# hritikbharucha/Custom_Porechop_ABI

Hardware: AMD Instinct MI355X
Metric: reads/sec trimmed (100k ONT reads x 50 adapter pairs) (higher is better)
Workload: dtype int32

## Files before the change

### __graft_entry__.py

```python
import os
import subprocess
import sys

ROOT = os.path.dirname(os.path.abspath(__file__))
PKG = os.path.join(ROOT, 'custom_porechop_abi_amd')
HIPCC = os.environ.get('HIPCC', '/opt/rocm/bin/hipcc')


def _run(cmd, **kw):
    print('+', ' '.join(cmd), flush=True)
    subprocess.check_call(cmd, **kw)


def build_lib():
    from concurrent.futures import ThreadPoolExecutor
    csrc = os.path.join(PKG, 'csrc')
    out = os.path.join(PKG, 'libpcabi.so')
    bdir = os.path.join(ROOT, 'build')
    os.makedirs(bdir, exist_ok=True)
    hdr = os.path.join(ROOT, 'include', 'pcabi.h')
    dp, kern = os.path.join(csrc, 'pcabi_dp.h'), os.path.join(csrc, 'pcabi_kern.h')
    hip = [HIPCC, '--offload-arch=gfx950', '-O3', '-std=c++17', '-fPIC', '-Wall', '-c']
    hostdev = os.path.join(csrc, 'pcabi_hostdev.h')
    host = [dp, kern, hdr, os.path.join(csrc, 'pcabi_host.h'), os.path.join(csrc, 'pcabi_scratch.h'), hostdev]
    units = [(name, host, hip) for name in ('pcabi_engine.hip', 'pcabi_hostapi.hip', 'pcabi_middle.hip', 'pcabi_seed.hip')]
    units += [(name, [dp, kern, hdr], hip) for name in
             ('pcabi_k_packed_small.hip', 'pcabi_k_packed_large.hip', 'pcabi_k_fast.hip',
              'pcabi_k_chunk.hip', 'pcabi_k_aux.hip', 'pcabi_k_split.hip', 'pcabi_k_split_chunk.hip',
              'pcabi_k_group.hip', 'pcabi_cuts.hip', 'pcabi_decide.hip', 'pcabi_paths.hip')]
    defl, crc = os.path.join(csrc, 'pcabi_deflate.h'), os.path.join(csrc, 'pcabi_crc.h')
    infl = os.path.join(csrc, 'pcabi_inflate.h')
    bam = os.path.join(csrc, 'pcabi_bam.h')
    units += [('pcabi_kmer.hip', [os.path.join(csrc, 'pcabi_kmer.h'), hdr], hip),
              ('pcabi_deflate.hip', [defl, crc, hostdev, hdr], hip),
              ('pcabi_inflate.hip', [infl, defl, crc, hostdev, hdr], hip),
              ('pcabi_gzstream.hip', [os.path.join(csrc, 'pcabi_gzstream.h'), infl, defl, crc, hostdev, hdr], hip),
              ('pcabi_bam.hip', [bam, hostdev, hdr], hip),
              ('pcabi_mods.hip', [os.path.join(csrc, 'pcabi_mods.h'), bam, hostdev, hdr], hip),
              ('pcabi_moves.hip', [os.path.join(csrc, 'pcabi_moves.h'), hostdev, hdr], hip),
              ('pcabi_qual.hip', [os.path.join(csrc, 'pcabi_qual.h'), os.path.join(csrc, 'pcabi_pieces.h'), hostdev, hdr], hip),
              ('pcabi_auxtext.hip', [os.path.join(csrc, 'pcabi_auxtext.h'), hostdev, hdr], hip),
              ('pcabi_auxparse.hip', [os.path.join(csrc, 'pcabi_auxparse.h'), hostdev, hdr], hip)]
    reads, gxx = os.path.join(csrc, 'pcabi_reads.h'), ['g++', '-O3', '-std=c++17', '-fPIC', '-Wall', '-c']
    units += [('pcabi_io.cpp', [bam, reads, hostdev, hdr], gxx),
              ('pcabi_write.cpp', [defl, bam, os.path.join(csrc, 'pcabi_auxtext.h'), reads, hostdev, hdr], gxx)]

    def stale(target, deps):
        return not os.path.isfile(target) or any(os.path.getmtime(target) < os.path.getmtime(d) for d in deps)

    def compile_unit(u):
        name, deps, cmd = u
        src = os.path.join(csrc, name)
        obj = os.path.join(bdir, os.path.splitext(name)[0] + '.o')
        if stale(obj, [src] + deps):
            _run(cmd + ['-o', obj + '.tmp', src])
            os.replace(obj + '.tmp', obj)
        return obj

    jobs = int(os.environ.get('PCABI_BUILD_JOBS', min(8, os.cpu_count() or 1)))
    with ThreadPoolExecutor(max_workers=jobs) as ex:
        objs = list(ex.map(compile_unit, units))
    if stale(out, objs):
        _run([HIPCC, '--offload-arch=gfx950', '-shared', '-fPIC', '-o', out + '.tmp'] + objs + ['-lz'])
        os.replace(out + '.tmp', out)
    return out


def build_pystr():
    import sysconfig
    src = os.path.join(PKG, 'csrc', 'pystr.c')
    out = os.path.join(PKG, '_pystr' + sysconfig.get_config_var('EXT_SUFFIX'))
    if not os.path.isfile(out) or os.path.getmtime(out) < os.path.getmtime(src):
        _run(['gcc', '-O2', '-shared', '-fPIC', '-Wall', '-I', sysconfig.get_paths()['include'], '-o', out + '.tmp', src])
        os.replace(out + '.tmp', out)
    return out


# ... 48 lines not shown
```

### custom_porechop_abi_amd/csrc/pcabi_engine.hip

```cpp
#include <hip/hip_runtime.h>

#include <algorithm>
#include <atomic>
#include <cstdio>
#include <cstdlib>
#include <cstring>
#include <mutex>
#include <string>
#include <thread>
#include <vector>

#include "../../include/pcabi.h"
#include "pcabi_dp.h"
#include "pcabi_kern.h"
#include "pcabi_host.h"

namespace {
thread_local std::string g_err;
}

namespace pcabi_eng {
int fail(int code, const std::string &msg) {
    g_err = msg;
    return code;
}
}

using namespace pcabi_eng;

namespace {


int bucket_of(int L, const pcabi::Scoring &sc, bool allow_wide = true) {
    if (L > kMaxRPL) return kStripedBucket;
    if (L <= 64) {
        const int rpl = (L + 3) & ~3;
        if (pcabi::fast_ok(L, rpl, sc)) return rpl / 4 - 1;
    } else if (allow_wide && L <= pcabi::pk::MAX_L) {
        const int rpl = (L + 3) & ~3;
        if (pcabi::packed_ok(L, rpl, sc)) return 16 + (rpl - 68) / 4;
    } else if (allow_wide && L <= pcabi::pk::MAX_L_LONG) {
        const int b = L <= 96 ? 22 : (L <= 112 ? 23 : 24);
        if (pcabi::long_ok(L, kBuckets[b].rpl, sc)) return b;
    }
    if (L > 64 && sc.go != sc.ge) return kStripedBucket;
    for (int b = 0; b < kNumBuckets; ++b)
        if (kBuckets[b].kind == GENERIC && L <= kBuckets[b].rpl) return b;
    return -1;
}


struct EndFields {
    int rs, re, m, l1;
};
__device__ __forceinline__ EndFields end_fields(const int32_t *res, int64_t stride, int64_t i) {
    return EndFields{res[0 * stride + i], res[1 * stride + i], res[5 * stride + i], res[6 * stride + i]};
}

__global__ __launch_bounds__(256) void k_end_trim(const int32_t *sres, int64_t sstride, int32_t n_sa,
                                                  const int32_t *eres, int64_t estride, int32_t n_ea,
                                                  int64_t n_read, int end_size, int extra,
                                                  double thr, int min_trim,
                                                  int32_t *start_trim, int32_t *end_trim,
                                                  uint8_t *shit, uint8_t *ehit) {
    __shared__ int s_st[4][64], s_et[4][64];
    const int lane = threadIdx.x & 63, w = threadIdx.x >> 6;
    const int64_t r = (int64_t)blockIdx.x * 64 + lane;
// ... 615 lines not shown
}
int pcabi_event_destroy(void *ev) { HIP_TRY(hipEventDestroy((hipEvent_t)ev)); return 0; }
int pcabi_event_record(void *ev, void *stream) { HIP_TRY(hipEventRecord((hipEvent_t)ev, (hipStream_t)stream)); return 0; }
int pcabi_stream_wait_event(void *stream, void *ev) {
    HIP_TRY(hipStreamWaitEvent((hipStream_t)stream, (hipEvent_t)ev, 0));
    return 0;
}
int pcabi_event_elapsed_ms(float *ms, void *start, void *stop) {
    HIP_TRY(hipEventSynchronize((hipEvent_t)stop));
    HIP_TRY(hipEventElapsedTime(ms, (hipEvent_t)start, (hipEvent_t)stop));
    return 0;
}

}

namespace {
int adapters_create_impl(const uint8_t *adp_codes, const int32_t *adp_off, const int32_t *adp_len,
                         int32_t n_adp, const pcabi::Scoring *sc, pcabi_adapters **out, bool all_striped = false) {
    if (int rc = check_adapter_lens(adp_len, n_adp)) return rc;
    BucketHost bk[kNumBuckets];
    build_buckets(adp_codes, adp_off, adp_len, n_adp, sc ? *sc : pcabi::Scoring{1, -1, -1, -1}, bk, sc != nullptr,
                  sc != nullptr, all_striped);
    pcabi_adapters *a = new pcabi_adapters();
    a->n_adp = n_adp;
    a->hoff.resize((size_t)n_adp);
    a->hlen.assign(adp_len, adp_len + n_adp);
    for (int k = 0; k < n_adp; ++k) {
        a->hoff[k] = (int32_t)a->hcodes.size();
        for (int i = 0; i < adp_len[k]; ++i) {
            if (adp_codes[adp_off[k] + i] > 3) a->has_n = true;
            a->hcodes.push_back(adp_codes[adp_off[k] + i]);
        }
    }
    for (int b = 0; b < kNumBuckets; ++b) {
        const int nb = (int)bk[b].len.size();
        a->count[b] = nb;
        if (!nb) continue;
        a->lens[b] = bk[b].len;
        a->ids[b] = bk[b].id;
        a->rt[b] = bk[b].rt;
        for (int k = 0; k < nb; ++k) {
            if (bk[b].len[k] != kBuckets[b].rpl) a->padded[b] = true;
            a->max_off[b] = std::max(a->max_off[b], kBuckets[b].rpl - bk[b].len[k]);
        }
        const int64_t nw = (int64_t)bk[b].pad.size() / 4;
        if (a->pad[b].reserve(nw, nw) || a->len[b].reserve(nb, nb) || a->id[b].reserve(nb, nb)) {
            pcabi_adapters_destroy(a);
            return fail(PCABI_E_NOMEM, "hipMalloc failed for adapter table");
        }
        (void)hipMemcpy(a->pad[b], bk[b].pad.data(), bk[b].pad.size(), hipMemcpyHostToDevice);
        (void)hipMemcpy(a->len[b], bk[b].len.data(), sizeof(int32_t) * nb, hipMemcpyHostToDevice);
        (void)hipMemcpy(a->id[b], bk[b].id.data(), sizeof(int32_t) * nb, hipMemcpyHostToDevice);
    }
    *out = a;
    return 0;
}
}

bool layout_serves(const pcabi_adapters *adps, const pcabi::Scoring &sc, int64_t max_win) {
    int max_L = 0;
    bool regs = false;
    for (int b = 0; b < kNumBuckets; ++b) {
        if (!adps->count[b] || kBuckets[b].kind == STRIPED) continue;
        regs = true;
        for (int32_t L : adps->lens[b]) max_L = std::max<int>(max_L, L);
        if (kBuckets[b].kind == FAST && adps->padded[b] && !pcabi::fast_ok(kBuckets[b].rpl - 1, kBuckets[b].rpl, sc))
            return false;
        if (kBuckets[b].kind == FAST && adps->max_off[b] > 3 && !bucket_packed_ok(b, adps->lens[b], sc)) return false;
        if (kBuckets[b].kind == WIDE || kBuckets[b].kind == LONG)
            for (int32_t L : adps->lens[b])
                if (kBuckets[b].kind == WIDE ? !pcabi::packed_ok(L, kBuckets[b].rpl, sc)
                                             : !pcabi::long_ok(L, kBuckets[b].rpl, sc))
                    return false;
    }
    return !regs || !needs_striped(sc, max_L, max_win);
}

int adapters_for(const pcabi_adapters *adps, const pcabi::Scoring &sc, int64_t max_win, const pcabi_adapters **use) {
    if (layout_serves(adps, sc, max_win)) {
        *use = adps;
        return 0;
    }
    pcabi_adapters *a = const_cast<pcabi_adapters *>(adps);
    std::lock_guard<std::mutex> g(a->alt_mu);
    std::vector<int32_t> off((size_t)a->n_adp);
    for (int32_t k = 0; k < a->n_adp; ++k) off[k] = a->hoff[k];
    pcabi_adapters *t = nullptr;
    for (auto &e : a->alt_scored)
        if (e.first.ma == sc.ma && e.first.mi == sc.mi && e.first.go == sc.go && e.first.ge == sc.ge) t = e.second;
    if (!t) {
        if (int rc = adapters_create_impl(a->hcodes.data(), off.data(), a->hlen.data(), a->n_adp, &sc, &t)) return rc;
        a->alt_scored.emplace_back(sc, t);
    }
    if (layout_serves(t, sc, max_win)) {
        *use = t;
        return 0;
    }
    if (!a->alt_striped) {
        t = nullptr;
        if (int rc = adapters_create_impl(a->hcodes.data(), off.data(), a->hlen.data(), a->n_adp, &sc, &t, true))
            return rc;
        a->alt_striped = t;
    }
    *use = a->alt_striped;
    return 0;
}

static int record_event(void *ev, hipStream_t st) {
    HIP_TRY(hipEventRecord((hipEvent_t)ev, st));
    return 0;
}

static int bucket_params(const pcabi_adapters *t, int b, const pcabi::Scoring &sc, KParams &p) {
    p.adp_pad = t->pad[b];
    p.adp_len = t->len[b];
    p.adp_id = t->id[b];
    p.n_adp = t->count[b];
    p.rt = t->rt[b];
    const int pack = bucket_pack_mode(b, t->lens[b], sc);
    bucket_shift(b, t->lens[b], sc, pack, p);
    return pack;
}

extern "C" {

int pcabi_adapters_create(const uint8_t *adp_codes, const int32_t *adp_off, const int32_t *adp_len,
                          int32_t n_adp, pcabi_adapters **out) {
    return adapters_create_impl(adp_codes, adp_off, adp_len, n_adp, nullptr, out);
}

int pcabi_adapters_create_scored(const uint8_t *adp_codes, const int32_t *adp_off, const int32_t *adp_len,
                                 int32_t n_adp, int match, int mismatch, int gap_open, int gap_extend,
                                 pcabi_adapters **out) {
    const pcabi::Scoring sc{match, mismatch, gap_open, gap_extend};
    return adapters_create_impl(adp_codes, adp_off, adp_len, n_adp, &sc, out);
}

void pcabi_adapters_destroy(pcabi_adapters *a) {
    if (!a) return;
    for (auto &e : a->alt_scored) pcabi_adapters_destroy(e.second);
    pcabi_adapters_destroy(a->alt_striped);
    delete a;
}

int64_t pcabi_tile_layout(const int32_t *win_len, int64_t n_win, int64_t *tile_off) {
    if (n_win < 0 || !win_len || !tile_off) return fail(PCABI_E_ARG, "bad arguments");
    return tile_layout(win_len, n_win, tile_off, nullptr);
}

int pcabi_tile_windows_dev(const uint8_t *codes, const int64_t *win_off, const int32_t *win_len,
                           int64_t n_win, const int64_t *tile_off, int64_t max_chunks, uint32_t *tiles,
                           void *stream) {
    if (n_win < 0) return fail(PCABI_E_ARG, "bad arguments");
    launch_tiles(codes, win_off, win_len, n_win, tile_off, max_chunks, tiles, (hipStream_t)stream);
    HIP_TRY(hipGetLastError());
    return 0;
}

int pcabi_align_cross_dev(const uint32_t *tiles, const int64_t *tile_off, const int32_t *win_len,
                          int64_t n_win, int32_t max_win_len, const pcabi_adapters *adps, int match,
                          int mismatch, int gap_open, int gap_extend, int32_t *out, int64_t out_stride,
                          void *stream) {
    return pcabi_align_cross_dev_marked(tiles, tile_off, win_len, n_win, max_win_len, adps, match, mismatch,
                                        gap_open, gap_extend, out, out_stride, stream, nullptr, nullptr);
}

int pcabi_align_cross_dev_marked(const uint32_t *tiles, const int64_t *tile_off, const int32_t *win_len,
                                 int64_t n_win, int32_t max_win_len, const pcabi_adapters *adps, int match,
                                 int mismatch, int gap_open, int gap_extend, int32_t *out, int64_t out_stride,
                                 void *stream, void *ev_begin, void *ev_end) {
    if (!adps || n_win < 0 || (n_win > 0 && (!tiles || !tile_off))) return fail(PCABI_E_ARG, "bad arguments");
    if (n_win == 0) return 0;
    if (int rc = adapters_for(adps, pcabi::Scoring{match, mismatch, gap_open, gap_extend}, max_win_len, &adps))
        return rc;
    KParams p{};
    p.tiles = tiles;
    p.tile_off = tile_off;
    p.win_len = win_len;
    p.n_win = n_win;
    p.out = out;
    p.out_stride = out_stride;
    p.sc = pcabi::Scoring{match, mismatch, gap_open, gap_extend};
    p.max_cols = max_win_len;
    const bool affine = gap_open != gap_extend;
    std::vector<int> order;
    for (int b = 0; b < kNumBuckets; ++b)
        if (adps->count[b]) order.push_back(b);
    std::stable_sort(order.begin(), order.end(), [&](int x, int y) {
        return (int64_t)adps->count[x] * kBuckets[x].rpl > (int64_t)adps->count[y] * kBuckets[y].rpl;
    });
    ForkJoin fj;
    if (int rc = fj.begin((hipStream_t)stream, order.size())) return rc;
    for (size_t k = 0; k < order.size(); ++k) {
        const int b = order[k];
        const int pack = bucket_params(adps, b, p.sc, p);
        const hipStream_t st = fj.at(k);
        int rc = k == 0 && ev_begin ? record_event(ev_begin, st) : 0;
        if (!rc) rc = dispatch(b, p, affine, st, pack);
        if (!rc && k == 0 && ev_end) rc = record_event(ev_end, st);
        if (rc) {
            (void)fj.end();
            return rc;
        }
    }
    if (int rc = fj.end()) return rc;
    HIP_TRY(hipGetLastError());
    return 0;
}

int pcabi_align_cross_multi_dev(const pcabi_cross_region *regions, int32_t n_regions, int match, int mismatch,
                                int gap_open, int gap_extend, void *stream, void *ev_begin, void *ev_end) {
    if (n_regions < 0 || (n_regions > 0 && !regions)) return fail(PCABI_E_ARG, "bad arguments");
    const pcabi::Scoring sc{match, mismatch, gap_open, gap_extend};
    const bool affine = gap_open != gap_extend;
    struct Unit {
        int cls, b, pack;
        KParams p;
        int64_t blocks, cost;
    };
    std::vector<Unit> units;
    for (int32_t r = 0; r < n_regions; ++r) {
        const pcabi_cross_region &g = regions[r];
        if (!g.adps || g.n_win < 0 || (g.n_win > 0 && (!g.tiles || !g.tile_off || !g.win_len || !g.out)))
            return fail(PCABI_E_ARG, "bad region " + std::to_string(r));
        if (g.n_win == 0) continue;
        const pcabi_adapters *adps = nullptr;
        if (int rc = adapters_for(g.adps, sc, g.max_win_len, &adps)) return rc;
        for (int b = 0; b < kNumBuckets; ++b) {
            if (!adps->count[b]) continue;
            Unit u{};
            u.b = b;
            KParams &p = u.p;
            p.tiles = g.tiles;
            p.tile_off = g.tile_off;
            p.win_len = g.win_len;
            p.n_win = g.n_win;
            p.out = g.out;
            p.out_stride = g.out_stride;
            p.sc = sc;
            p.max_cols = g.max_win_len;
            u.pack = bucket_params(adps, b, sc, p);
            u.cls = kBuckets[b].kind == FAST ? group_class(kBuckets[b].rpl, u.pack, affine) : -1;
            u.blocks = (g.n_win + 8 * 256 - 1) / (8 * 256) * 8 * (int64_t)p.n_adp;
            u.cost = (g.n_win + 255) / 256 * (int64_t)p.n_adp * kBuckets[b].rpl;
            units.push_back(u);
        }
    }
    if (units.empty()) return 0;
    struct Launch {
        int cls;
        size_t unit;
        GroupParams gp;
        int64_t blocks, cost;
    };
    std::vector<Launch> launches;
    for (int c = 0; c < kGroupClasses; ++c) {
        std::vector<size_t> mine;
        for (size_t k = 0; k < units.size(); ++k)
            if (units[k].cls == c) mine.push_back(k);
        if (mine.size() == 1) units[mine[0]].cls = -1;
        if (mine.size() <= 1) continue;
        std::stable_sort(mine.begin(), mine.end(),
                         [&](size_t x, size_t y) { return kBuckets[units[x].b].rpl > kBuckets[units[y].b].rpl; });
        for (size_t k0 = 0; k0 < mine.size(); k0 += kMaxGroupSegs) {
            Launch l{};
            l.cls = c;
            l.gp.sc = sc;
            for (size_t k = k0; k < std::min(mine.size(), k0 + kMaxGroupSegs); ++k) {
                const Unit &u = units[mine[k]];
                GroupSeg &s = l.gp.seg[l.gp.n_seg++];
                s.tiles = u.p.tiles;
                s.tile_off = u.p.tile_off;
                s.win_len = u.p.win_len;
                s.n_win = u.p.n_win;
                s.adp_pad = u.p.adp_pad;
                s.adp_len = u.p.adp_len;
                s.adp_id = u.p.adp_id;
                s.n_adp = u.p.n_adp;
                s.out = u.p.out;
                s.out_stride = u.p.out_stride;
                s.rpl = kBuckets[u.b].rpl;
                s.shift_p = u.p.shift_p;
                s.shift_b = u.p.shift_b;
                s.block0 = l.blocks;
                l.blocks += u.blocks;
                l.cost += u.cost;
            }
            launches.push_back(l);
        }
    }
    for (size_t k = 0; k < units.size(); ++k)
        if (units[k].cls < 0) {
            Launch l{};
            l.cls = -1;
            l.unit = k;
            l.cost = units[k].cost;
            launches.push_back(l);
        }
    std::stable_sort(launches.begin(), launches.end(), [](const Launch &x, const Launch &y) { return x.cost > y.cost; });
    ForkJoin fj;
    if (int rc = fj.begin((hipStream_t)stream, launches.size())) return rc;
    for (size_t k = 0; k < launches.size(); ++k) {
        const Launch &l = launches[k];
        const hipStream_t st = fj.at(k);
        int rc = k == 0 && ev_begin ? record_event(ev_begin, st) : 0;
        if (!rc && l.cls >= 0) dispatch_group(l.cls, l.gp, l.blocks, st);
        else if (!rc) rc = dispatch(units[l.unit].b, units[l.unit].p, affine, st, units[l.unit].pack);
        if (!rc && k == 0 && ev_end) rc = record_event(ev_end, st);
        if (rc) {
            (void)fj.end();
            return rc;
        }
    }
    if (int rc = fj.end()) return rc;
    HIP_TRY(hipGetLastError());
    return 0;
}

int pcabi_set_side_streams(int on) {
    const int prev = side_streams_on() ? 1 : 0;
    if (on >= 0) g_side_on.store(on ? 1 : 0);
    return prev;
}

int pcabi_stream_side_streams(void *stream, int on) {
    const hipStream_t st = (hipStream_t)stream;
    std::lock_guard<std::mutex> g(g_stream_side_mu);
    for (size_t k = 0; k < g_stream_side.size(); ++k)
        if (g_stream_side[k].first == st) {
            const int prev = g_stream_side[k].second;
// ... 58 lines not shown
```

### custom_porechop_abi_amd/csrc/pcabi_host.h

```cpp
#pragma once

#include <hip/hip_runtime.h>

#include <atomic>
#include <mutex>
#include <utility>
#include <vector>

#include "../../include/pcabi.h"
#include "pcabi_dp.h"
#include "pcabi_kern.h"
#include "pcabi_scratch.h"

using pcabi_internal::Scratch;

void pcabi_poison_async(void *p, size_t bytes, hipStream_t st);

extern std::atomic<uint64_t> g_table_serial;
struct pcabi_adapters {
    int32_t n_adp = 0;
    uint64_t serial = g_table_serial.fetch_add(1) + 1;
    int rt[pcabi_eng::kNumBuckets] = {};
    bool padded[pcabi_eng::kNumBuckets] = {};
    int max_off[pcabi_eng::kNumBuckets] = {};
    std::vector<int32_t> lens[pcabi_eng::kNumBuckets];
    std::vector<int32_t> ids[pcabi_eng::kNumBuckets];
    bool has_n = false;
    std::vector<uint8_t> hcodes;
    std::vector<int32_t> hoff, hlen;
    int32_t count[pcabi_eng::kNumBuckets] = {};
    pcabi_internal::DevBuf<uint32_t> pad[pcabi_eng::kNumBuckets];
    pcabi_internal::DevBuf<int32_t> len[pcabi_eng::kNumBuckets], id[pcabi_eng::kNumBuckets];
    std::mutex alt_mu;
    std::vector<std::pair<pcabi::Scoring, pcabi_adapters *>> alt_scored;
    pcabi_adapters *alt_striped = nullptr;
};
bool layout_serves(const pcabi_adapters *adps, const pcabi::Scoring &sc, int64_t max_win);
int adapters_for(const pcabi_adapters *adps, const pcabi::Scoring &sc, int64_t max_win, const pcabi_adapters **use);

namespace pcabi_eng {

struct SideStreams;
struct ForkJoin {
    hipStream_t main = nullptr;
    SideStreams *ss = nullptr;
    std::unique_lock<std::mutex> lock;
    int first = 0;
    unsigned used = 0;
    int n_side = 0;
    int begin(hipStream_t m, size_t n_launch);
    hipStream_t at(size_t k);
    int end();
};

int64_t tile_layout(const int32_t *win_len, int64_t n_win, int64_t *tile_off, int64_t *max_nq);
void launch_tiles(const uint8_t *codes, const int64_t *win_off, const int32_t *win_len, int64_t n_win,
                  const int64_t *tile_off, int64_t max_nq, uint32_t *tiles, hipStream_t st);
int first_hit_from(const int32_t *res, int64_t stride, int64_t n_win, int32_t n_adp, double threshold,
                   const int32_t *start_adp, int32_t *hits, int64_t hit_stride, hipStream_t st);
void scan_set_table(pcabi_scan *s, const pcabi_adapters *adps);
bool chunkable(int b, bool packed);
int dispatch(int b, const KParams &p, bool affine, hipStream_t st, int packed);
bool bucket_packed_ok(int b, const std::vector<int32_t> &lens, const pcabi::Scoring &sc);
int bucket_pack_mode(int b, const std::vector<int32_t> &lens, const pcabi::Scoring &sc);
void bucket_shift(int b, const std::vector<int32_t> &lens, const pcabi::Scoring &sc, int pack_mode, KParams &p);

struct BucketHost {
    std::vector<uint8_t> pad;
    std::vector<int32_t> len, id;
    int rt = 0;
};
void build_buckets(const uint8_t *adp_codes, const int32_t *adp_off, const int32_t *adp_len, int32_t n_adp,
                   const pcabi::Scoring &sc, BucketHost (&bk)[kNumBuckets], bool merge = true, bool allow_wide = true,
                   bool all_striped = false);
int check_adapter_lens(const int32_t *adp_len, int32_t n_adp);
bool needs_striped(const pcabi::Scoring &sc, int max_L, int64_t max_win);

}

namespace pcabi_seed {
struct State;
State *create();
void destroy(State *s);
int bounds(State *s, const void *adps_key, const uint8_t *hcodes, const int32_t *hoff, const int32_t *hlen,
           int32_t n_adp, const std::vector<int> &fb_rows, const uint8_t *codes, const int64_t *v_off,
// ... 22 lines not shown
```

### custom_porechop_abi_amd/csrc/pcabi_k_group.hip

```cpp
#include "pcabi_kern.h"

namespace pcabi_eng {

template <int CLS>
__global__ __launch_bounds__(256) void k_align_group(GroupParams gp) {
    constexpr int MAXR = group_max_rpl(CLS);
    __shared__ __attribute__((aligned(16))) int32_t tab[4 * kTabW * MAXR];
    int32_t *wave_tab = tab + (threadIdx.x >> 6) * kTabW * MAXR;
    const int64_t b = blockIdx.x;
    int s = 0;
    while (s + 1 < gp.n_seg && b >= gp.seg[s + 1].block0) ++s;
    const GroupSeg &g = gp.seg[s];
    KParams p{};
    p.tiles = g.tiles;
    p.tile_off = g.tile_off;
    p.win_len = g.win_len;
    p.n_win = g.n_win;
    p.adp_pad = g.adp_pad;
    p.adp_len = g.adp_len;
    p.adp_id = g.adp_id;
    p.n_adp = g.n_adp;
    p.out = g.out;
    p.out_stride = g.out_stride;
    p.sc = gp.sc;
    p.shift_p = g.shift_p;
    p.shift_b = g.shift_b;
    const int64_t lb = b - g.block0;
    if constexpr (CLS == 0) {
        if (g.shift_p > 0) {
            switch (g.rpl) {
#define T(R) case R: cross_block<R, true, SHIFT>(p, lb, wave_tab); break;
            T(4) T(8) T(12) T(16) T(20) T(24) T(28) T(32)
#undef T
            }
        } else {
            switch (g.rpl) {
#define T(R) case R: cross_block<R, true, TAGGED>(p, lb, wave_tab); break;
            T(4) T(8) T(12) T(16) T(20) T(24) T(28) T(32)
#undef T
            }
        }
    } else {
        if (g.shift_p > 0) {
            switch (g.rpl) {
#define P(R) case R: cross_block<R, true, PSHIFT>(p, lb, wave_tab); break;
            P(36) P(40) P(44) P(48) P(52) P(56) P(60) P(64)
#undef P
            }
        } else {
            switch (g.rpl) {
#define P(R) case R: cross_block<R, true, PACKED>(p, lb, wave_tab); break;
            P(36) P(40) P(44) P(48) P(52) P(56) P(60) P(64)
#undef P
            }
        }
    }
}

void dispatch_group(int cls, const GroupParams &p, int64_t blocks, hipStream_t st) {
    if (blocks <= 0) return;
    if (cls == 0) hipLaunchKernelGGL((k_align_group<0>), dim3((unsigned)blocks), dim3(256), 0, st, p);
    else hipLaunchKernelGGL((k_align_group<1>), dim3((unsigned)blocks), dim3(256), 0, st, p);
}

}
```

### custom_porechop_abi_amd/csrc/pcabi_kern.h

```cpp
#pragma once
#include <hip/hip_runtime.h>

#include <algorithm>
#include <cstdint>
#include <cstdlib>
#include <string>
#include <type_traits>

#include "../../include/pcabi.h"
#include "pcabi_dp.h"

#ifndef PCABI_WAVES
#define PCABI_WAVES 1
#endif

void pcabi_poison(void *p, size_t bytes);
void pcabi_poison_async(void *p, size_t bytes, hipStream_t st);

namespace pcabi_eng {

int fail(int code, const std::string &msg);

#define HIP_TRY(expr)                                                                   \
    do {                                                                                \
        hipError_t e_ = (expr);                                                         \
        if (e_ != hipSuccess)                                                           \
            return fail(PCABI_E_DEVICE, std::string(#expr) + ": " + hipGetErrorString(e_)); \
    } while (0)

enum Kind { FAST = 0, GENERIC = 1, PACKED = 2, WIDE = 3, LONG = 4, STRIPED = 5,
            TAGGED = 6,
            SHIFT = 7,
            PSHIFT = 8 };
struct BucketDef {
    int rpl;
    Kind kind;
};
constexpr BucketDef kBuckets[] = {
    {4, FAST},  {8, FAST},  {12, FAST}, {16, FAST}, {20, FAST}, {24, FAST}, {28, FAST}, {32, FAST},
    {36, FAST}, {40, FAST}, {44, FAST}, {48, FAST}, {52, FAST}, {56, FAST}, {60, FAST}, {64, FAST},
    {68, WIDE}, {72, WIDE}, {76, WIDE}, {80, WIDE}, {84, WIDE}, {88, WIDE},
    {96, LONG}, {112, LONG}, {128, LONG},
    {16, GENERIC}, {32, GENERIC}, {64, GENERIC}, {96, GENERIC}, {128, GENERIC},
    {256, STRIPED}};
constexpr int kNumBuckets = sizeof(kBuckets) / sizeof(kBuckets[0]);
constexpr int kStripedBucket = kNumBuckets - 1;
constexpr int kMaxRPL = 128;
constexpr int kStripeRows = 32;
constexpr int kStripeTab = 64;

struct KParams {
    const uint8_t *codes;
    const int64_t *win_off;
    const int32_t *win_len;
    int64_t n_win;
    const uint32_t *tiles;
    const int64_t *tile_off;
    const uint32_t *adp_pad;
    const int32_t *adp_len;
    const int32_t *adp_id;
    int32_t n_adp;
    const int32_t *task_win;
    const int32_t *task_out;
    const int32_t *wave_adp;
    int64_t n_waves;
    int32_t *out;
    int64_t out_stride;
    pcabi::Scoring sc;
    int32_t *compat;
    int32_t chunk_split;
    const int4 *task_chunk;
    int32_t rt;
    int32_t max_cols;
    int32_t *scratch;
    int64_t n_items;
    const int32_t *dev_waves;
    int32_t shift_p, shift_b;
};

struct WindowReader {
    const uint32_t *q;
    int64_t stride;
    int a8;
    uint32_t lo, hi, nx;
    __device__ __forceinline__ WindowReader() : q(nullptr), stride(0), a8(0), lo(0), hi(0), nx(0) {}
    __device__ __forceinline__ WindowReader(const uint32_t *base, int64_t stride_, int a8_)
        : q(base), stride(stride_), a8(a8_) {
        lo = q[0]; hi = q[stride]; nx = q[2 * stride];
    }
    __device__ __forceinline__ int operator()(int j) {
        const int k = j - 1;
        if (k > 0 && (k & 3) == 0) { lo = hi; hi = nx; nx = q[(int64_t)(k / 4 + 2) * stride]; }
        return (int)(((((uint64_t)hi << 32) | lo) >> (8 * (k & 3) + a8)) & 0xFFu);
    }
};

template <int RPL>
struct AdapterRegs {
    uint32_t w[RPL / 4];
    __device__ __forceinline__ void load(const uint32_t *src) {
#pragma unroll
        for (int k = 0; k < RPL / 4; ++k) w[k] = __builtin_amdgcn_readfirstlane(src[k]);
    }
    __device__ __forceinline__ int operator()(int s) const {
        return (int)((w[(s - 1) >> 2] >> (8 * ((s - 1) & 3))) & 0xFFu);
    }
};

__device__ __forceinline__ void store_result(int32_t *out, int64_t stride, int64_t idx,
                                             const pcabi::Result &r) {
    out[0 * stride + idx] = r.rs;
    out[1 * stride + idx] = r.re;
    out[2 * stride + idx] = r.as;
    out[3 * stride + idx] = r.ae;
    out[4 * stride + idx] = r.score;
    out[5 * stride + idx] = r.m;
    out[6 * stride + idx] = r.l1;
    out[7 * stride + idx] = r.l2;
}

__device__ __forceinline__ pcabi::Result empty_result() {
    pcabi::Result r;
    r.rs = -1; r.re = 0; r.as = -1; r.ae = 0;
    r.score = (int)0x80000000; r.m = 0; r.l1 = 0; r.l2 = 0;
    return r;
}

constexpr int kTabW = pcabi::pk::TAB_W;

struct LdsRow {
    const int32_t *p;
    __device__ __forceinline__ int32_t operator()(int s) const { return p[s - 1]; }
    __device__ __forceinline__ void quad(int q, int32_t *dst) const {
        const int4 v = *reinterpret_cast<const int4 *>(p + 4 * q);
        dst[0] = v.x; dst[1] = v.y; dst[2] = v.z; dst[3] = v.w;
    }
};

template <int RPL, typename Y = pcabi::pk::Lay<RPL>>
__device__ __forceinline__ void fill_wave_tab(const KParams &p, int a_local, int L, int32_t *wave_tab) {
    const int off = RPL - L;
    const int lane = threadIdx.x & 63;
    for (int e = lane; e < kTabW * RPL; e += 64) {
        const int c = e / RPL, srow = e % RPL + 1;
        const uint32_t *ap = p.adp_pad + (int64_t)a_local * (RPL / 4);
        auto code = [&](int sl) { return (int)((ap[(sl - 1) / 4] >> (8 * ((sl - 1) & 3))) & 0xFFu); };
        wave_tab[e] = pcabi::pk::sub_key<RPL, decltype(code), Y>(srow, c, code, off, p.sc);
    }
    __syncthreads();
}

template <int RPL>
__device__ __forceinline__ void fill_wave_tab_shift(const KParams &p, int a_local, int L, int32_t *wave_tab) {
    const int off = RPL - L;
    const int lane = threadIdx.x & 63;
    for (int e = lane; e < kTabW * RPL; e += 64) {
        const int c = e / RPL, srow = e % RPL + 1;
        const uint32_t *ap = p.adp_pad + (int64_t)a_local * (RPL / 4);
        auto code = [&](int sl) { return (int)((ap[(sl - 1) / 4] >> (8 * ((sl - 1) & 3))) & 0xFFu); };
        wave_tab[e] = pcabi::pk::sub_key_shift<RPL>(srow, c, code, off, p.sc);
    }
    __syncthreads();
}

template <int RPL>
__device__ __forceinline__ void fill_wave_tab_pshift(const KParams &p, int a_local, int L, int32_t *wave_tab) {
    const int off = RPL - L;
    const int lane = threadIdx.x & 63;
    for (int e = lane; e < kTabW * RPL; e += 64) {
        const int c = e / RPL, srow = e % RPL + 1;
        const uint32_t *ap = p.adp_pad + (int64_t)a_local * (RPL / 4);
// ... 43 lines not shown
            auto tr = [&](int q) { return base[(int64_t)q * 256]; };
            auto tabfn = [&](int rc) { return LdsRow{wave_tab + rc * RPL}; };
            r = pcabi::align_lane_shift4<RPL>(tr, n0, tabfn, L, p.sc, P, p.shift_b);
            uniform = true;
        }
    }
    if (uniform) {
    } else if (n <= 0) {
        r = empty_result();
    } else {
        WindowReader rd = tile_off >= 0
            ? WindowReader(p.tiles + tile_off + (threadIdx.x & 255), 256, 0)
            : [&] {
                  const uint8_t *b = p.codes + p.win_off[w];
                  const int a0 = (int)((uintptr_t)b & 3);
                  return WindowReader(reinterpret_cast<const uint32_t *>(b - a0), 1, 8 * a0);
              }();
        if constexpr (KIND == PACKED) {
            auto tabfn = [&](int rc) { return LdsRow{wave_tab + rc * RPL}; };
            r = pcabi::align_lane_packed<(RPL <= pcabi::pk::MAX_RPL ? RPL : 4), AFFINE>(rd, n, tabfn, L, p.sc);
        } else if constexpr (KIND == TAGGED) {
            static_assert(RPL <= 32 && AFFINE, "run-tagged layout: affine buckets of <= 32 rows");
            auto tabfn = [&](int rc) { return LdsRow{wave_tab + rc * RPL}; };
            r = pcabi::align_lane_packed<RPL, true, false, pcabi::pk::LayT<RPL>>(rd, n, tabfn, L, p.sc);
        } else if constexpr (KIND == SHIFT) {
            static_assert(RPL <= 32 && AFFINE, "gap-extend frame: affine buckets of <= 32 rows");
            auto tabfn = [&](int rc) { return LdsRow{wave_tab + rc * RPL}; };
            r = pcabi::align_lane_shift<RPL>(rd, n, tabfn, L, p.sc, p.shift_p, p.shift_b);
        } else if constexpr (KIND == PSHIFT) {
            static_assert(RPL >= 36 && RPL <= 64 && AFFINE, "packed gap-extend frame: affine buckets of 36..64 rows");
            auto tabfn = [&](int rc) { return LdsRow{wave_tab + rc * RPL}; };
            r = pcabi::align_lane_pshift<RPL>(rd, n, tabfn, L, p.sc, p.shift_p, p.shift_b);
        } else if constexpr (KIND == LONG) {
            WindowReader rd1 = rd;
            auto tab0 = [&](int rc) { return LdsRow{wave_tab + rc * RPL}; };
            auto tab1 = [&](int rc) { return LdsRow{wave_tab + kTabW * RPL + rc * RPL}; };
            r = pcabi::align_lane_packed_long<RPL, AFFINE>(rd, rd1, n, tab0, tab1, L, p.sc);
        } else if constexpr (KIND == FAST) {
            r = pcabi::align_lane_fast<RPL, AFFINE>(rd, n, adp, L, p.sc);
        } else {
            r = pcabi::align_lane_generic<RPL, AFFINE>(rd, n, adp, L, p.sc);
        }
    }
    if (p.compat) {
        int en_match = 0;
        if (r.rs >= 0 && r.diag_en && r.l1 > 0) {
            const uint8_t *ab = reinterpret_cast<const uint8_t *>(p.adp_pad + (int64_t)a_local * (RPL / 4));
            en_match = p.codes[p.win_off[w] + r.re] == ab[RPL - L + r.ae];
        }
        p.compat[out_idx] = pcabi::compat_flag(r, n, en_match);
        return;
    }
    store_result(p.out, p.out_stride, out_idx, r);
}

template <int KIND, int RPL>
constexpr int wave_tab_ints() {
    return (KIND == PACKED || KIND == TAGGED || KIND == SHIFT || KIND == PSHIFT) ? kTabW * RPL : (KIND == LONG ? 2 * kTabW * RPL : 1);
}

template <int RPL, bool AFFINE, int KIND>
__device__ __forceinline__ void cross_block(const KParams &p, int64_t b, int32_t *wave_tab) {
    const int64_t k = b >> 3;
    const int a_local = (int)(k % p.n_adp);
    const int64_t tile = (k / p.n_adp) * 8 + (b & 7);
    const int64_t w = tile * 256 + threadIdx.x;
    const int a_glob = p.adp_id[a_local];
    const int64_t toff = w < p.n_win ? p.tile_off[tile] : 0;
    run_lane<RPL, AFFINE, KIND>(p, a_local, w < p.n_win ? w : -1, (int64_t)a_glob * p.n_win + w, wave_tab, toff);
}

template <int RPL, bool AFFINE, int KIND>
__global__ __launch_bounds__(256, PCABI_WAVES) void k_align(KParams p) {
    __shared__ __attribute__((aligned(16))) int32_t tab[4 * wave_tab_ints<KIND, RPL>()];
    int32_t *wave_tab = tab + (threadIdx.x >> 6) * wave_tab_ints<KIND, RPL>();
    if (p.task_win == nullptr) {
        cross_block<RPL, AFFINE, KIND>(p, blockIdx.x, wave_tab);
    } else {
        int64_t wave = (int64_t)blockIdx.x * 4 + (threadIdx.x >> 6);
        const bool live = wave < p.n_waves;
        if (!live) wave = p.n_waves - 1;
        const int64_t slot = wave * 64 + (threadIdx.x & 63);
        const int a_local = __builtin_amdgcn_readfirstlane(p.wave_adp[wave]);
        const int32_t tw = live ? p.task_win[slot] : -1;
        run_lane<RPL, AFFINE, KIND>(p, a_local, tw, tw >= 0 ? p.task_out[slot] : 0, wave_tab, -1);
    }
}

struct FParams {
    const uint32_t *tiles;
    const int64_t *tile_off;
    const int32_t *win_len;
    int64_t n_win;
    const uint32_t *adp_pad;
    const int32_t *adp_len;
    const int32_t *adp_id;
    int32_t n_adp;
    int16_t *s16;
    pcabi::Scoring sc;
};

struct LdsRow16 {
    const int32_t *p;
    __device__ __forceinline__ void quad(int q, pcabi::sf::v2 *dst) const {
        const int4 v = *reinterpret_cast<const int4 *>(p + 4 * q);
        dst[0] = __builtin_bit_cast(pcabi::sf::v2, v.x);
// ... 139 lines not shown

template <int R, bool AFFINE>
__global__ __launch_bounds__(256) void k_align_striped(KParams p) {
    const int64_t slot = (int64_t)blockIdx.x * 4 + (threadIdx.x >> 6);
    const int lane = threadIdx.x & 63;
    const int64_t n_slots = (int64_t)gridDim.x * 4;
    StripeBnd<AFFINE> bnd{p.scratch + slot * (int64_t)p.max_cols * (StripeBnd<AFFINE>::NF * 64) + lane};
    for (int64_t item = slot; item < p.n_items; item += n_slots) {
        const bool cross = p.task_win == nullptr;
        int a_local;
        int64_t w, out_idx, q = 0;
        int4 ck = make_int4(0, 0, 1, -1);
        if (cross) {
            a_local = (int)(item % p.n_adp);
            q = item / p.n_adp;
            w = q * 64 + lane;
            if (w >= p.n_win) continue;
            out_idx = (int64_t)p.adp_id[a_local] * p.n_win + w;
        } else {
            a_local = p.wave_adp[item];
            const int64_t sl = item * 64 + lane;
            w = p.task_win[sl];
            if (w < 0) continue;
            out_idx = p.task_out[sl];
            if (p.task_chunk) ck = p.task_chunk[sl];
        }
        a_local = __builtin_amdgcn_readfirstlane(a_local);
        const int L = __builtin_amdgcn_readfirstlane(p.adp_len[a_local]);
        const int n = p.task_chunk ? ck.y : p.win_len[w];
        pcabi::Result r;
        if (n <= 0) {
            r = empty_result();
        } else {
            WindowReader rd = cross
                ? WindowReader(p.tiles + p.tile_off[q >> 2] + (q & 3) * 64 + lane, 256, 0)
                : [&] {
                      const uint8_t *b = p.codes + p.win_off[w] + ck.x;
                      const int a0 = (int)((uintptr_t)b & 3);
                      return WindowReader(reinterpret_cast<const uint32_t *>(b - a0), 1, 8 * a0);
                  }();
            StripeAdp<R> adp{p.adp_pad + (int64_t)a_local * (p.rt / 4)};
            r = pcabi::align_lane_striped<R, AFFINE>(rd, n, adp, L, p.rt, p.sc, bnd, ck.z, ck.w);
        }
        if (p.compat) {
            int en_match = 0;
            if (r.rs >= 0 && r.diag_en && r.l1 > 0) {
                const uint8_t *ab = reinterpret_cast<const uint8_t *>(p.adp_pad + (int64_t)a_local * (p.rt / 4));
                en_match = p.codes[p.win_off[w] + r.re] == ab[p.rt - L + r.ae];
            }
            p.compat[out_idx] = pcabi::compat_flag(r, n, en_match);
            continue;
        }
        store_result(p.out, p.out_stride, out_idx, r);
    }
}

__device__ __forceinline__ int32_t lane_from_below(int32_t v) {
    return __builtin_amdgcn_update_dpp(0, v, 0x111, 0xF, 0xF, false);
}

template <int RPL, int K, bool AFFINE, int KIND>
__global__ __launch_bounds__(256, PCABI_WAVES) void k_align_split(KParams p) {
    constexpr int R = RPL / K;
    static_assert(RPL % K == 0 && 16 % K == 0 && R >= 2, "split geometry");
    using Y = typename std::conditional<KIND == TAGGED, pcabi::pk::LayT<RPL>, pcabi::pk::Lay<RPL>>::type;
    __shared__ __attribute__((aligned(16))) int32_t tab[4 * kTabW * RPL];
    int32_t *wave_tab = tab + (threadIdx.x >> 6) * (kTabW * RPL);
    const int64_t b = blockIdx.x;
    const int64_t k = b >> 3;
    const int a_local = (int)(k % p.n_adp);
    const int64_t q = k / p.n_adp;
    const int64_t tile = (q / K) * 8 + (b & 7);
    const int l = (int)(threadIdx.x % K);
    const int64_t w = tile * 256 + (q % K) * (256 / K) + threadIdx.x / K;
    const int L = __builtin_amdgcn_readfirstlane(p.adp_len[a_local]);
    fill_wave_tab<RPL, Y>(p, a_local, L, wave_tab);
    const bool live = w < p.n_win;
    const int n = live ? p.win_len[w] : 0;
    int nmax = n;
#pragma unroll
    for (int o = 1; o < 64; o <<= 1) nmax = max(nmax, __shfl_xor(nmax, o));
    WindowReader rd;
    if (n > 0) rd = WindowReader(p.tiles + p.tile_off[tile] + (w & 255), 256, 0);
    pcabi::LaneSplit<R, AFFINE, Y> st;
    st.init(l, K, L, RPL, p.sc);
    int32_t sg = st.gbot, sv = st.vbot;
    const int steps = nmax - 1 + K - 1;
#pragma unroll 1
    for (int t = 1; t <= steps; ++t) {
        int32_t rg = lane_from_below(sg), rv = lane_from_below(sv);
        if (l == 0) {
            rg = st.row0_g(t);
            rv = st.neg2;
        }
        const int j = t - l;
        if (j >= 1 && j < n) {
            const int c = rd(j);
            st.inner(LdsRow{wave_tab + c * RPL + st.r0}, j, rg, rv);
            sg = st.gbot;
            sv = st.vbot;
        }
    }
    st.out = pcabi::SplitIn{};
#pragma unroll
    for (int ph = 0; ph < K; ++ph) {
        pcabi::SplitIn in;
        in.gup = lane_from_below(st.out.gup);
        in.vup = lane_from_below(st.out.vup);
        in.slt = lane_from_below(st.out.slt);
        in.vt = lane_from_below(st.out.vt);
        in.vp = lane_from_below(st.out.vp);
        in.score = lane_from_below(st.out.score);
        in.bi = lane_from_below(st.out.bi);
        in.lt = lane_from_below(st.out.lt);
        in.trail = lane_from_below(st.out.trail);
        in.prec = lane_from_below(st.out.prec);
        in.attr = (uint32_t)lane_from_below((int32_t)st.out.attr);
        if (l == ph && n > 0) {
            if (l == 0) in = st.empty_in(n);
            const int c = rd(n);
            st.last_col(LdsRow{wave_tab + c * RPL + st.r0}, n, in);
        }
    }
    if (l == K - 1 && live)
        store_result(p.out, p.out_stride, (int64_t)p.adp_id[a_local] * p.n_win + w, n > 0 ? st.result(n) : empty_result());
}

template <int RPL, int K, bool AFFINE, int KIND>
__device__ __forceinline__ void split_chunk_wave(const KParams &p, int64_t pw, int sub, bool live, int32_t *wave_tab) {
    constexpr int R = RPL / K;
    using Y = typename std::conditional<KIND == TAGGED, pcabi::pk::LayT<RPL>, pcabi::pk::Lay<RPL>>::type;
    const int lane = threadIdx.x & 63, l = lane % K;
    const int64_t slot = pw * 64 + sub * (64 / K) + lane / K;
    const int a_local = __builtin_amdgcn_readfirstlane(p.wave_adp[pw]);
    const int L = __builtin_amdgcn_readfirstlane(p.adp_len[a_local]);
    fill_wave_tab<RPL, Y>(p, a_local, L, wave_tab);
    const int32_t tw = live ? p.task_win[slot] : -1;
    int4 ck = make_int4(0, 0, 1, 0);
    if (tw >= 0) ck = p.task_chunk[slot];
    const int n = tw >= 0 ? ck.y : 0;
    const bool at_end = ck.w < 0;
    const int hi = at_end ? n + 1 : ck.w;
    const int n_in = at_end ? n - 1 : n;
    int nmax = n_in;
#pragma unroll
    for (int o = 1; o < 64; o <<= 1) nmax = max(nmax, __shfl_xor(nmax, o));
    WindowReader rd;
    if (n > 0) {
        const uint8_t *b = p.codes + p.win_off[tw] + ck.x;
        const int a0 = (int)((uintptr_t)b & 3);
        rd = WindowReader(reinterpret_cast<const uint32_t *>(b - a0), 1, 8 * a0);
    }
    pcabi::LaneSplit<R, AFFINE, Y> st;
    st.init(l, K, L, RPL, p.sc);
    int32_t sg = st.gbot, sv = st.vbot;
    const int steps = nmax + K - 1;
#pragma unroll 1
    for (int t = 1; t <= steps; ++t) {
        int32_t rg = lane_from_below(sg), rv = lane_from_below(sv);
        if (l == 0) {
            rg = st.row0_g(t);
            rv = st.neg2;
        }
        const int j = t - l;
        if (j >= 1 && j <= n_in) {
            const int c = rd(j);
            st.inner(LdsRow{wave_tab + c * RPL + st.r0}, j, rg, rv, j >= ck.z && j < hi);
            sg = st.gbot;
            sv = st.vbot;
        }
    }
    st.out = pcabi::SplitIn{};
#pragma unroll
    for (int ph = 0; ph < K; ++ph) {
        pcabi::SplitIn in;
        in.gup = lane_from_below(st.out.gup);
        in.vup = lane_from_below(st.out.vup);
        in.slt = lane_from_below(st.out.slt);
        in.vt = lane_from_below(st.out.vt);
        in.vp = lane_from_below(st.out.vp);
        in.score = lane_from_below(st.out.score);
        in.bi = lane_from_below(st.out.bi);
        in.lt = lane_from_below(st.out.lt);
        in.trail = lane_from_below(st.out.trail);
        in.prec = lane_from_below(st.out.prec);
        in.attr = (uint32_t)lane_from_below((int32_t)st.out.attr);
        if (l == ph && n > 0 && at_end) {
            if (l == 0) in = st.empty_in(n);
            const int c = rd(n);
            st.last_col(LdsRow{wave_tab + c * RPL + st.r0}, n, in);
        }
    }
    if (!at_end) st.materialize();
    if (l == K - 1 && tw >= 0)
        store_result(p.out, p.out_stride, p.task_out[slot], n > 0 ? st.result(at_end ? n : n + 1) : empty_result());
}

template <int RPL, int K, bool AFFINE, int KIND>
__global__ __launch_bounds__(256) void k_align_split_chunk(KParams p) {
    static_assert(RPL % K == 0 && 16 % K == 0 && RPL / K >= 2, "split geometry");
    __shared__ __attribute__((aligned(16))) int32_t tab[4 * kTabW * RPL];
    int32_t *wave_tab = tab + (threadIdx.x >> 6) * (kTabW * RPL);
    const int64_t w0 = p.dev_waves[0], nsub = (int64_t)p.dev_waves[1] * K;
    for (int64_t wb = blockIdx.x; wb * 4 < nsub; wb += gridDim.x) {
        int64_t sw = wb * 4 + (threadIdx.x >> 6);
        const bool live = sw < nsub;
        if (!live) sw = nsub - 1;
        split_chunk_wave<RPL, K, AFFINE, KIND>(p, w0 + sw / K, (int)(sw % K), live, wave_tab);
    }
}

template <int RPL, int KIND>
void launch(const KParams &p, bool affine, dim3 grid, hipStream_t st) {
    if (affine) hipLaunchKernelGGL((k_align<RPL, true, KIND>), grid, dim3(256), 0, st, p);
    else hipLaunchKernelGGL((k_align<RPL, false, KIND>), grid, dim3(256), 0, st, p);
}

constexpr int kMaxGroupSegs = 16;
constexpr int kGroupClasses = 2;
struct GroupSeg {
    const uint32_t *tiles;
    const int64_t *tile_off;
    const int32_t *win_len;
    int64_t n_win;
    const uint32_t *adp_pad;
    const int32_t *adp_len;
    const int32_t *adp_id;
    int32_t *out;
    int64_t out_stride;
    int64_t block0;
    int32_t n_adp;
    int32_t rpl;
    int32_t shift_p, shift_b;
};
struct GroupParams {
    GroupSeg seg[kMaxGroupSegs];
    int32_t n_seg;
    pcabi::Scoring sc;
};
constexpr int group_max_rpl(int cls) { return cls == 0 ? 32 : 64; }
inline int group_class(int rpl, int pack_mode, bool affine) {
    if (!affine) return -1;
    if (pack_mode == 2 && rpl <= 32) return 0;
    if (pack_mode == 1 && rpl >= 36 && rpl <= 64) return 1;
    return -1;
}
void dispatch_group(int cls, const GroupParams &p, int64_t blocks, hipStream_t st);

constexpr int kMaxChunkSegs = 8;
constexpr int kChunkGroupRpl = 28;
struct ChunkSeg {
    const uint32_t *adp_pad;
    const int32_t *adp_len;
    const int32_t *adp_id;
    const int32_t *dev_waves;
    int32_t n_adp;
    int32_t rpl;
};
struct ChunkGroupParams {
    KParams p;
    ChunkSeg seg[kMaxChunkSegs];
    int32_t n_seg;
};
void dispatch_chunk_group(const ChunkGroupParams &gp, unsigned blocks, hipStream_t st);

void dispatch_packed_small(int rpl, const KParams &p, bool affine, dim3 grid, hipStream_t st, bool tagged);
void dispatch_packed_large(int rpl, bool long_kind, const KParams &p, bool affine, dim3 grid,
                           hipStream_t st);
void dispatch_fast(int rpl, bool generic, const KParams &p, bool affine, dim3 grid, hipStream_t st);
int dispatch_chunk(int b, const KParams &p, bool affine, hipStream_t st, bool tagged = false);
void dispatch_filter(int rpl, const FParams &p, bool affine, hipStream_t st);
bool dispatch_split(int rpl, int K, const KParams &p, bool affine, bool tagged, hipStream_t st);
bool dispatch_split_chunk(int rpl, int K, const KParams &p, bool affine, bool tagged, hipStream_t st);
int launch_striped(KParams p, bool affine, hipStream_t st);

}
```

Measured before the change: 17.44 million.

## Deduplicate identical adapter sequences and fan out alignment results to aliases

At adapter-table build time, identical adapter sequences are grouped and per-bucket reduced tables containing only one representative per group are uploaded. Kernels align only the representatives and then copy each result to the output slots of the duplicate adapters by following an alias linked list. This removes redundant DP work when the adapter set contains repeated sequences. The cost is extra host-side grouping, extra device tables, and serial alias stores in the kernel epilogue. Some kernel paths (chunked task path) skip alias stores, which risks missing outputs in those paths.

After: 17.56 million (median of 6 runs). No clear change (+0.7%).

```diff
diff --git a/__graft_entry__.py b/__graft_entry__.py
--- a/__graft_entry__.py
+++ b/__graft_entry__.py
@@ -22,7 +22,8 @@
     dp, kern = os.path.join(csrc, 'pcabi_dp.h'), os.path.join(csrc, 'pcabi_kern.h')
     hip = [HIPCC, '--offload-arch=gfx950', '-O3', '-std=c++17', '-fPIC', '-Wall', '-c']
     hostdev = os.path.join(csrc, 'pcabi_hostdev.h')
-    host = [dp, kern, hdr, os.path.join(csrc, 'pcabi_host.h'), os.path.join(csrc, 'pcabi_scratch.h'), hostdev]
+    host = [dp, kern, hdr, os.path.join(csrc, 'pcabi_host.h'), os.path.join(csrc, 'pcabi_alias.h'),
+            os.path.join(csrc, 'pcabi_scratch.h'), hostdev]
     units = [(name, host, hip) for name in ('pcabi_engine.hip', 'pcabi_hostapi.hip', 'pcabi_middle.hip', 'pcabi_seed.hip')]
     units += [(name, [dp, kern, hdr], hip) for name in
              ('pcabi_k_packed_small.hip', 'pcabi_k_packed_large.hip', 'pcabi_k_fast.hip',
diff --git a/custom_porechop_abi_amd/csrc/pcabi_alias.h b/custom_porechop_abi_amd/csrc/pcabi_alias.h
--- /dev/null
+++ b/custom_porechop_abi_amd/csrc/pcabi_alias.h
@@ -0,0 +1,36 @@
+#pragma once
+
+#include <cstdint>
+#include <cstring>
+#include <vector>
+
+namespace pcabi_alias {
+
+struct Groups {
+    std::vector<int32_t> kept;
+    std::vector<int32_t> next;
+    bool any() const { return kept.size() != next.size(); }
+};
+
+inline Groups group_identical(const uint8_t *codes, const int32_t *off, const int32_t *len, int32_t n) {
+    Groups g;
+    g.next.assign((size_t)(n > 0 ? n : 0), -1);
+    std::vector<int32_t> tail;
+    for (int32_t k = 0; k < n; ++k) {
+        size_t j = 0;
+        for (; j < g.kept.size(); ++j) {
+            const int32_t f = g.kept[j];
+            if (len[f] == len[k] && (len[k] <= 0 || std::memcmp(codes + off[f], codes + off[k], (size_t)len[k]) == 0)) break;
+        }
+        if (j == g.kept.size()) {
+            g.kept.push_back(k);
+            tail.push_back(k);
+        } else {
+            g.next[(size_t)tail[j]] = k;
+            tail[j] = k;
+        }
+    }
+    return g;
+}
+
+}
diff --git a/custom_porechop_abi_amd/csrc/pcabi_engine.hip b/custom_porechop_abi_amd/csrc/pcabi_engine.hip
--- a/custom_porechop_abi_amd/csrc/pcabi_engine.hip
+++ b/custom_porechop_abi_amd/csrc/pcabi_engine.hip
@@ -13,6 +13,7 @@
 #include "../../include/pcabi.h"
 #include "pcabi_dp.h"
 #include "pcabi_kern.h"
+#include "pcabi_alias.h"
 #include "pcabi_host.h"
 
 namespace {
@@ -734,6 +735,38 @@
         (void)hipMemcpy(a->len[b], bk[b].len.data(), sizeof(int32_t) * nb, hipMemcpyHostToDevice);
         (void)hipMemcpy(a->id[b], bk[b].id.data(), sizeof(int32_t) * nb, hipMemcpyHostToDevice);
     }
+    const pcabi_alias::Groups grp = pcabi_alias::group_identical(adp_codes, adp_off, adp_len, n_adp);
+    if (grp.any()) {
+        std::vector<uint8_t> is_kept((size_t)n_adp, 0);
+        for (int32_t k : grp.kept) is_kept[(size_t)k] = 1;
+        bool bad = a->alias.reserve(n_adp, n_adp) != 0;
+        if (!bad) (void)hipMemcpy(a->alias, grp.next.data(), sizeof(int32_t) * n_adp, hipMemcpyHostToDevice);
+        for (int b = 0; b < kNumBuckets && !bad; ++b) {
+            const int nb = a->count[b];
+            const size_t row = nb ? bk[b].pad.size() / (size_t)nb : 0;
+            std::vector<uint8_t> pad;
+            std::vector<int32_t> len, id;
+            for (int k = 0; k < nb; ++k) {
+                if (!is_kept[(size_t)bk[b].id[k]]) continue;
+                pad.insert(pad.end(), bk[b].pad.begin() + (long)(k * row), bk[b].pad.begin() + (long)((k + 1) * row));
+                len.push_back(bk[b].len[k]);
+                id.push_back(bk[b].id[k]);
+            }
+            const int nx = (int)id.size();
+            a->xcount[b] = nx;
+            if (nx == nb || nx == 0) continue;
+            const int64_t nw = (int64_t)pad.size() / 4;
+            bad = a->xpad[b].reserve(nw, nw) || a->xlen[b].reserve(nx, nx) || a->xid[b].reserve(nx, nx);
+            if (bad) break;
+            (void)hipMemcpy(a->xpad[b], pad.data(), pad.size(), hipMemcpyHostToDevice);
+            (void)hipMemcpy(a->xlen[b], len.data(), sizeof(int32_t) * nx, hipMemcpyHostToDevice);
+            (void)hipMemcpy(a->xid[b], id.data(), sizeof(int32_t) * nx, hipMemcpyHostToDevice);
+        }
+        if (bad) {
+            pcabi_adapters_destroy(a);
+            return fail(PCABI_E_NOMEM, "hipMalloc failed for adapter table");
+        }
+    }
     *out = a;
     return 0;
 }
@@ -798,6 +831,13 @@
     p.adp_len = t->len[b];
     p.adp_id = t->id[b];
     p.n_adp = t->count[b];
+    p.adp_alias = t->alias;
+    if (t->alias && t->xcount[b] < t->count[b]) {
+        p.adp_pad = t->xpad[b];
+        p.adp_len = t->xlen[b];
+        p.adp_id = t->xid[b];
+        p.n_adp = t->xcount[b];
+    }
     p.rt = t->rt[b];
     const int pack = bucket_pack_mode(b, t->lens[b], sc);
     bucket_shift(b, t->lens[b], sc, pack, p);
@@ -878,7 +918,7 @@
         const int pack = bucket_params(adps, b, p.sc, p);
         const hipStream_t st = fj.at(k);
         int rc = k == 0 && ev_begin ? record_event(ev_begin, st) : 0;
-        if (!rc) rc = dispatch(b, p, affine, st, pack);
+        if (!rc && p.n_adp > 0) rc = dispatch(b, p, affine, st, pack);
         if (!rc && k == 0 && ev_end) rc = record_event(ev_end, st);
         if (rc) {
             (void)fj.end();
@@ -922,6 +962,7 @@
             p.sc = sc;
             p.max_cols = g.max_win_len;
             u.pack = bucket_params(adps, b, sc, p);
+            if (p.n_adp == 0) continue;
             u.cls = kBuckets[b].kind == FAST ? group_class(kBuckets[b].rpl, u.pack, affine) : -1;
             u.blocks = (g.n_win + 8 * 256 - 1) / (8 * 256) * 8 * (int64_t)p.n_adp;
             u.cost = (g.n_win + 255) / 256 * (int64_t)p.n_adp * kBuckets[b].rpl;
@@ -958,6 +999,7 @@
                 s.adp_pad = u.p.adp_pad;
                 s.adp_len = u.p.adp_len;
                 s.adp_id = u.p.adp_id;
+                s.adp_alias = u.p.adp_alias;
                 s.n_adp = u.p.n_adp;
                 s.out = u.p.out;
                 s.out_stride = u.p.out_stride;
diff --git a/custom_porechop_abi_amd/csrc/pcabi_host.h b/custom_porechop_abi_amd/csrc/pcabi_host.h
--- a/custom_porechop_abi_amd/csrc/pcabi_host.h
+++ b/custom_porechop_abi_amd/csrc/pcabi_host.h
@@ -31,6 +31,10 @@
     int32_t count[pcabi_eng::kNumBuckets] = {};
     pcabi_internal::DevBuf<uint32_t> pad[pcabi_eng::kNumBuckets];
     pcabi_internal::DevBuf<int32_t> len[pcabi_eng::kNumBuckets], id[pcabi_eng::kNumBuckets];
+    int32_t xcount[pcabi_eng::kNumBuckets] = {};
+    pcabi_internal::DevBuf<uint32_t> xpad[pcabi_eng::kNumBuckets];
+    pcabi_internal::DevBuf<int32_t> xlen[pcabi_eng::kNumBuckets], xid[pcabi_eng::kNumBuckets];
+    pcabi_internal::DevBuf<int32_t> alias;
     std::mutex alt_mu;
     std::vector<std::pair<pcabi::Scoring, pcabi_adapters *>> alt_scored;
     pcabi_adapters *alt_striped = nullptr;
diff --git a/custom_porechop_abi_amd/csrc/pcabi_k_group.hip b/custom_porechop_abi_amd/csrc/pcabi_k_group.hip
--- a/custom_porechop_abi_amd/csrc/pcabi_k_group.hip
+++ b/custom_porechop_abi_amd/csrc/pcabi_k_group.hip
@@ -19,6 +19,7 @@
     p.adp_pad = g.adp_pad;
     p.adp_len = g.adp_len;
     p.adp_id = g.adp_id;
+    p.adp_alias = g.adp_alias;
     p.n_adp = g.n_adp;
     p.out = g.out;
     p.out_stride = g.out_stride;
diff --git a/custom_porechop_abi_amd/csrc/pcabi_kern.h b/custom_porechop_abi_amd/csrc/pcabi_kern.h
--- a/custom_porechop_abi_amd/csrc/pcabi_kern.h
+++ b/custom_porechop_abi_amd/csrc/pcabi_kern.h
@@ -59,6 +59,7 @@
     const uint32_t *adp_pad;
     const int32_t *adp_len;
     const int32_t *adp_id;
+    const int32_t *adp_alias;
     int32_t n_adp;
     const int32_t *task_win;
     const int32_t *task_out;
@@ -117,6 +118,14 @@
     out[5 * stride + idx] = r.m;
     out[6 * stride + idx] = r.l1;
     out[7 * stride + idx] = r.l2;
+}
+
+__device__ __forceinline__ void store_aliases(const KParams &p, int a_local, int64_t out_idx, const pcabi::Result &r) {
+    if (p.adp_alias == nullptr) return;
+    const int a0 = __builtin_amdgcn_readfirstlane(p.adp_id[a_local]);
+    for (int a = __builtin_amdgcn_readfirstlane(p.adp_alias[a0]); a >= 0;
+         a = __builtin_amdgcn_readfirstlane(p.adp_alias[a]))
+        store_result(p.out, p.out_stride, out_idx + (int64_t)(a - a0) * p.n_win, r);
 }
 
 __device__ __forceinline__ pcabi::Result empty_result() {
@@ -266,6 +275,7 @@
         return;
     }
     store_result(p.out, p.out_stride, out_idx, r);
+    if (p.task_win == nullptr) store_aliases(p, a_local, out_idx, r);
 }
 
 template <int KIND, int RPL>
@@ -511,6 +521,7 @@
             continue;
         }
         store_result(p.out, p.out_stride, out_idx, r);
+        if (cross) store_aliases(p, a_local, out_idx, r);
     }
 }
 
@@ -581,8 +592,12 @@
             st.last_col(LdsRow{wave_tab + c * RPL + st.r0}, n, in);
         }
     }
-    if (l == K - 1 && live)
-        store_result(p.out, p.out_stride, (int64_t)p.adp_id[a_local] * p.n_win + w, n > 0 ? st.result(n) : empty_result());
+    if (l == K - 1 && live) {
+        const pcabi::Result r = n > 0 ? st.result(n) : empty_result();
+        const int64_t out_idx = (int64_t)p.adp_id[a_local] * p.n_win + w;
+        store_result(p.out, p.out_stride, out_idx, r);
+        store_aliases(p, a_local, out_idx, r);
+    }
 }
 
 template <int RPL, int K, bool AFFINE, int KIND>
@@ -685,6 +700,7 @@
     const uint32_t *adp_pad;
     const int32_t *adp_len;
     const int32_t *adp_id;
+    const int32_t *adp_alias;
     int32_t *out;
     int64_t out_stride;
     int64_t block0;
```
